# visinf/da-sac

Measured on AMD Instinct MI355X. Metric: train images/sec (769x769, 19-cls, RN101 DeepLabv2, K=3), higher is better.
Workload: dtype f32

## Files before the change

### da-sac_amd/csrc/conv_plan.hpp

```cpp
#pragma once
#include <cstddef>
#include <cstdint>

#include "chip.hpp"

#if defined(__HIPCC__)
#include <hip/hip_runtime.h>
#define DASAC_PLAN_HD __host__ __device__ __forceinline__
#else
#define DASAC_PLAN_HD inline
#endif

namespace dasac {

constexpr int kBK = 16;
constexpr int kSkWorkersPerCu = 3;
constexpr int kSkWorkers = kNumCu * kSkWorkersPerCu;
constexpr int kTileSlots = kNumCu * 4;
constexpr int kTailSlots = 2048;
constexpr int kTailMinSteps = 8;
constexpr double kTailPieceCost = 6.0;
constexpr int kTailMaxSplit = 8;
constexpr size_t kDepositBytes = (size_t)128 * 128 * sizeof(float);
constexpr size_t kPartialBytes = (size_t)(kTailSlots > kSkWorkers ? kTailSlots : kSkWorkers) * kDepositBytes;
constexpr size_t kGemmWorkspaceBytes = kPartialBytes + (size_t)(kTailSlots + 1) * sizeof(int);

constexpr int kWgPix = 32;
constexpr int kWgMinPix = 256;
constexpr int kWgSlots = kNumCu * 3;
constexpr int kWgMaxSplits = 64;
constexpr int kWgFewTiles = 12;
constexpr int kWgManyPix = 200000;
constexpr int64_t kMaxTensorBytes = (1ll << 32) - 4096;

inline int conv_mpad(int M) { return M > 64 ? (M + 127) / 128 * 128 : (M > 32 ? 64 : 32); }
inline int conv_kpad(int K) { return (K + 127) / 128 * 128; }
inline int pick_bm(int Mpad) { return Mpad % 128 == 0 ? 128 : (Mpad % 64 == 0 ? 64 : 32); }
DASAC_PLAN_HD int round_up_xcd(int n) { return (n + kNumXcd - 1) / kNumXcd * kNumXcd; }

inline int sk_workers(int reserved) { return (kNumCu - reserved) * kSkWorkersPerCu; }

inline bool want_streamk(int tiles, int k_steps, int reserved) {
  if ((long long)tiles * k_steps < sk_workers(reserved)) return false;
  const int resident = (kNumCu - reserved) * 3;
  const int rounds = (tiles + resident - 1) / resident;
  const double eff = (double)tiles / ((double)rounds * resident);
  return k_steps >= 64 ? eff < 0.93 : (k_steps >= 16 && eff < 0.6);
}

inline int tail_plan(int m_tiles, int n_tiles, int k_steps, int reserved, int& lead_n) {
  const int tiles = m_tiles * n_tiles;
  if (!want_streamk(tiles, k_steps, reserved)) return 0;
  lead_n = (tiles / kTileSlots) * kTileSlots / m_tiles;
// ... 95 lines not shown
  p.bm = pick_bm(p.Mpad);
  p.bnk = (M % 8 == 0 && p.bm != 32) ? wgrad_bn(Cx) : 128;
  p.m_tiles = p.Mpad / p.bm;
  p.k_tiles = p.Kpad / p.bnk;
  p.splits = wgrad_splits(p.Mpad, p.Kpad, Npix, p.bm, p.bnk);
  p.per = wgrad_per(Npix, p.splits);
  p.grid = round_up_xcd(p.m_tiles * p.k_tiles * p.splits);
  p.slab = (size_t)p.Mpad * p.Kpad;
  p.psum_offset = (size_t)p.splits * p.slab;
  const int s128 = wgrad_splits(p.Mpad, p.Kpad, Npix, p.bm, 128), s64 = wgrad_splits(p.Mpad, p.Kpad, Npix, p.bm, 64);
  p.workspace_bytes = (size_t)(s128 > s64 ? s128 : s64) * p.Mpad * (p.Kpad + 1) * sizeof(float);
  return p;
}

struct WgradBatchedPlan {
  int m_tiles, k_tiles, splits, per, grid;
  size_t psum_offset, workspace_bytes;
};
inline WgradBatchedPlan wgrad_batched_plan(int batch, int M, int C, int T) {
  WgradBatchedPlan p{};
  if (batch < 1 || batch > 65535 || M <= 0 || C <= 0 || T <= 0 || M % 128 || C % 128 || T % 4) return p;
  if ((int64_t)M * T * 4 >= (1ll << 31) || (int64_t)C * T * 4 >= (1ll << 31)) return p;
  if ((int64_t)batch * M * C * 4 > kMaxTensorBytes) return p;
  const int splits = wgrad_splits(batch * (M / 128) * (C / 128), T, kWgMaxSplits);
  if ((int64_t)splits * batch * M * C * 4 > kMaxTensorBytes) return p;
  p.m_tiles = M / 128;
  p.k_tiles = C / 128;
  p.splits = splits;
  p.per = wgrad_per(T, splits);
  p.grid = round_up_xcd(p.m_tiles * p.k_tiles * splits);
  p.psum_offset = (size_t)splits * batch * M * C;
  p.workspace_bytes = (size_t)splits * ((size_t)batch * M * C + M) * sizeof(float);
  return p;
}

struct GemmWork {
  bool has_work;
  int it, it_end;
};

DASAC_PLAN_HD GemmWork gemm_tile_work(int bid, int m_tiles, int n_tiles, int KT) {
  const int xcd = bid % kNumXcd, slot = bid / kNumXcd;
  const int per_xcd = (n_tiles + kNumXcd - 1) / kNumXcd;
  const int n_local = slot / m_tiles;
  const int n_tile = xcd * per_xcd + n_local;
  const int it = (n_tile * m_tiles + slot % m_tiles) * KT;
  return GemmWork{!(n_local >= per_xcd || n_tile >= n_tiles), it, it + KT};
// ... 25 lines not shown
```

### da-sac_amd/csrc/winograd.hip

```cpp
#include "conv_common.hpp"
#include "winograd_index.hpp"

namespace dasac {
namespace wino {

constexpr int kBlock = 256;

__device__ __forceinline__ float ld(__amdgpu_buffer_rsrc_t r, unsigned voff) {
  return __uint_as_float(__builtin_amdgcn_raw_buffer_load_b32(r, voff, 0, 0));
}
__device__ __forceinline__ void st(__amdgpu_buffer_rsrc_t r, unsigned voff, float v) {
  __builtin_amdgcn_raw_buffer_store_b32(__float_as_uint(v), r, voff, 0, 0);
}

struct F2 {
  static constexpr int TM = 2, N = TM + 2, P = kPoints<TM>;
  static constexpr bool kPaddedT = wino::kPaddedT<TM>;
  static __device__ __forceinline__ void bt(const float (&d)[4], float (&o)[4]) {
    o[0] = d[0] - d[2];
    o[1] = d[1] + d[2];
    o[2] = d[2] - d[1];
    o[3] = d[1] - d[3];
  }
  static __device__ __forceinline__ void a(const float (&y)[2], float (&o)[4]) {
// ... 33 lines not shown
    o[2] = (y[0] + y[2]) - (y[1] + y[3]);
    o[3] = (y[0] + 4.f * y[2]) + (2.f * y[1] + 8.f * y[3]);
    o[4] = (y[0] + 0.25f * y[2]) - (0.5f * y[1] + 0.125f * y[3]);
    o[5] = y[3];
  }
  static __device__ __forceinline__ void g(const float (&w)[3], float (&o)[6]) {
    o[0] = 0.5f * w[0];
    o[1] = k6 * ((w[0] + w[2]) + w[1]);
    o[2] = k6 * ((w[0] + w[2]) - w[1]);
    o[3] = (k30 * w[0] + k15 * w[1]) + (2.f * k15) * w[2];
    o[4] = ((16.f * k15) * w[0] - (8.f * k15) * w[1]) + (4.f * k15) * w[2];
    o[5] = 0.5f * w[2];
  }
  static __device__ __forceinline__ void gt(const float (&p)[6], float (&o)[3]) {
    o[0] = (0.5f * p[0] + k6 * (p[1] + p[2])) + (k30 * p[3] + (16.f * k15) * p[4]);
    o[1] = k6 * (p[1] - p[2]) + (k15 * p[3] - (8.f * k15) * p[4]);
    o[2] = (k6 * (p[1] + p[2]) + 0.5f * p[5]) + ((2.f * k15) * p[3] + (4.f * k15) * p[4]);
  }
  static __device__ __forceinline__ void at(const float (&y)[6], float (&o)[4]) {
    o[0] = (y[0] + (y[1] + y[2])) + (y[3] + y[4]);
    o[1] = (y[1] - y[2]) + (2.f * y[3] - 0.5f * y[4]);
    o[2] = (y[1] + y[2]) + (4.f * y[3] + 0.25f * y[4]);
    o[3] = ((y[1] - y[2]) + y[5]) + (8.f * y[3] - 0.125f * y[4]);
  }
};


template <class F>
__global__ __launch_bounds__(kBlock) void filter_transform(const float* __restrict__ Wt, const float* __restrict__ scale,
                                                            float* __restrict__ U, int Cout, int Cin, int Mpad, int Kpad, int mode,
                                                            unsigned w_bytes, unsigned u_bytes) {
  const int idx = blockIdx.x * kBlock + threadIdx.x;
  const int per_point = Kpad * Mpad;
  if (idx >= per_point) return;
  const __amdgpu_buffer_rsrc_t rw = make_rsrc(Wt, w_bytes), ru = make_rsrc(U, u_bytes);
  const int row4 = Mpad * 4;
  const int kq = idx / row4, rem = idx - kq * row4;
  const int m = rem >> 2, k = kq * 4 + (rem & 3);
  const int M = mode == 0 ? Cout : Cin, K = mode == 0 ? Cin : Cout;
  const bool real = m < M && k < K;
  const int co = mode == 0 ? m : k, ci = mode == 0 ? k : m;
  const float s = (real && scale) ? ld(make_rsrc(scale, (unsigned)Cout * 4u), (unsigned)co * 4u) : 1.f;
  float w[3][3];
#pragma unroll
  for (int a = 0; a < 3; ++a)
#pragma unroll
// ... 143 lines not shown
      float o[3];
      F::gt(r[a], o);
#pragma unroll
      for (int b = 0; b < 3; ++b) grad[c * 9 + a * 3 + b] = o[b];
    }
  }
  __syncthreads();
  const float sc = scale ? ld(make_rsrc(scale, (unsigned)M * 4u), (unsigned)co * 4u) : 1.f;
  float part = 0.f;
  for (int e = tx; e < 64 * 9; e += kBlock) {
    const unsigned off = ((unsigned)(co * C + ci0) * 9u + (unsigned)e) * 4u;
    if (dot) part += grad[e] * ld(rw, off);
    st(rd, off, grad[e] * sc);
  }
  if (dot) {
    __shared__ float redd[4];
    part = wave_sum(part);
    if (c == 0) redd[q] = part;
    __syncthreads();
    if (tx == 0) st(make_rsrc(dot, (unsigned)((C / 64) * M) * 4u), (unsigned)(blockIdx.x * M + co) * 4u, (redd[0] + redd[1]) + (redd[2] + redd[3]));
  }
}


__device__ __forceinline__ void record_bits(unsigned* obits, unsigned bits_bytes, int m, int w32, int pix, bool positive) {
  const unsigned long long ballot = __builtin_amdgcn_ballot_w64(positive);
  const int lane = threadIdx.x & 63, wcol = pix >> 5;
  if ((lane & 31) == 0 && wcol < w32)
    __builtin_amdgcn_raw_buffer_store_b32((unsigned)(lane ? ballot >> 32 : ballot), make_rsrc(obits, bits_bytes), out_bits_offset(m, w32, pix), 0, 0);
}

template <int BITS>
__global__ __launch_bounds__(kBlock) void output_transform(const float* __restrict__ Y, float* __restrict__ Out, Geom g, int M,
                                                            const float* __restrict__ shift, int relu,
                                                            const unsigned* __restrict__ mbits, unsigned* __restrict__ obits,
                                                            int w32, unsigned y_bytes, unsigned out_bytes, unsigned bits_bytes) {
  const int pix = blockIdx.x * kBlock + threadIdx.x;
  const int m = blockIdx.y;
  const bool live = pix < g.N * g.HW;
  const __amdgpu_buffer_rsrc_t ry = make_rsrc(Y, y_bytes), ro = make_rsrc(Out, out_bytes);
  int n = 0, rem = 0, tile = 0, ey = 0, ex = 0;
  if (live) pixel_tile(g, pix, n, rem, tile, ey, ex);
  float v[3][3];
#pragma unroll
  for (int j = 0; j < 3; ++j)
#pragma unroll
// ... 56 lines not shown
        v = (word >> (pix & 31)) & 1u ? v : 0.f;
      }
      st(ro, in ? out_offset(g, M, n, m, rem) : kOutside, v);
    }
  }
}

__global__ __launch_bounds__(kBlock) void relu_bits_pack(const float* __restrict__ Out, unsigned* __restrict__ obits, Geom g, int M,
                                                          int w32, unsigned out_bytes, unsigned bits_bytes) {
  const int pix = blockIdx.x * kBlock + threadIdx.x;
  const int m = blockIdx.y;
  const bool live = pix < g.N * g.HW;
  const int n = live ? div(pix, g.by_hw) : 0;
  const float v = ld(make_rsrc(Out, out_bytes), live ? out_offset(g, M, n, m, pix - n * g.HW) : kOutside);
  record_bits(obits, bits_bytes, m, w32, pix, live && v > 0.f);
}

}
}

using namespace dasac;
using dasac::wino::F2;
using dasac::wino::F4;
using dasac::wino::Geom;

template <class F>
static int wino_geom(Geom& g, const char* who, int Nb, int C, int H, int W, int dilation) {
  DASAC_REQUIRE(Nb > 0 && C > 0 && H > 0 && W > 0 && dilation > 0, "%s: bad geometry", who);
  DASAC_REQUIRE((int64_t)Nb * H * W < (1ll << 30), "%s: more than 2^30 pixels", who);
  g = wino::make_geom<F::TM>(Nb, H, W, dilation);
  DASAC_REQUIRE(F::P * (int64_t)C * g.T * 4 <= wino::kMaxBytes && (int64_t)C * Nb * H * W * 4 <= wino::kMaxBytes,
                "%s: a tensor exceeds the 4 GiB buffer-descriptor window", who);
  DASAC_REQUIRE(C <= 65535, "%s: more than 65535 channels", who);
  return DASAC_OK;
}

template <class F>
static int tiles_impl(int Nb, int H, int W, int dilation) {
  if (Nb <= 0 || H <= 0 || W <= 0 || dilation <= 0) return 0;
  const int64_t t = (int64_t)Nb * wino::make_axis<F::TM>(H, dilation).tiles * wino::make_axis<F::TM>(W, dilation).tiles;
  return t < (1ll << 30) ? (int)wino::padded_tiles<F::TM>(t) : 0;
}

template <class F>
static int filter_impl(const char* who, const float* w, const float* scale, int Cout, int Cin, int transposed, float* u,
                       dasac_stream_t stream) {
// ... 61 lines not shown
                         out_bytes, bits_bytes);
    if (relu_bits_out) {
      DASAC_CHECK_LAUNCH(who);
      hipLaunchKernelGGL(wino::relu_bits_pack, per_pixel, block, 0, s, out, relu_bits_out, g, M, w32, out_bytes, bits_bytes);
    }
  }
  DASAC_CHECK_LAUNCH(who);
  return DASAC_OK;
}

template <class F>
static int wgrad_finish_impl(const char* who, const void* workspace, size_t ws_bytes, int M, int C, int T, const float* w,
                             const float* scale, float* dw, float* dot, float* sum_dz, dasac_stream_t stream) {
  DASAC_REQUIRE(workspace && w && dw, "%s: null pointer", who);
  DASAC_REQUIRE(M > 0 && M <= 65535 && C > 0 && C % 64 == 0, "%s: needs 1..65535 output channels and a multiple of 64 input channels", who);
  const int splits = dasac_conv_wgrad_batched_splits(F::P, M, C, T);
  DASAC_REQUIRE(splits > 0, "%s: the batched weight-gradient launch does not take this shape", who);
  const size_t need = dasac_conv_wgrad_batched_workspace(F::P, M, C, T);
  if (ws_bytes < need) return fail(DASAC_EWORKSPACE, "%s: workspace too small (%zu < %zu)", who, ws_bytes, need);
  const int64_t s_elems = (int64_t)splits * F::P * M * C;
  DASAC_REQUIRE(s_elems * 4 <= wino::kMaxBytes && (int64_t)M * C * 9 * 4 <= wino::kMaxBytes,
                "%s: a tensor exceeds the 4 GiB buffer-descriptor window", who);
  const float* S = reinterpret_cast<const float*>(workspace);
  hipLaunchKernelGGL(wino::wgrad_finish<F>, dim3(C / 64, M), dim3(wino::kBlock), 0, as_stream(stream), S, S + s_elems, splits, M, C, w, scale,
                     dw, dot, sum_dz, (unsigned)(s_elems * 4), (unsigned)((int64_t)M * C * 9 * 4));
  DASAC_CHECK_LAUNCH(who);
  return DASAC_OK;
}

extern "C" int dasac_winograd_tiles(int Nb, int H, int W, int dilation) { return tiles_impl<F2>(Nb, H, W, dilation); }
extern "C" int dasac_winograd4_tiles(int Nb, int H, int W, int dilation) { return tiles_impl<F4>(Nb, H, W, dilation); }

extern "C" int dasac_winograd_filter(const float* w, const float* scale, int Cout, int Cin, int transposed, float* u,
                                     dasac_stream_t stream) {
  return filter_impl<F2>("winograd_filter", w, scale, Cout, Cin, transposed, u, stream);
}
extern "C" int dasac_winograd4_filter(const float* w, const float* scale, int Cout, int Cin, int transposed, float* u,
                                      dasac_stream_t stream) {
  return filter_impl<F4>("winograd4_filter", w, scale, Cout, Cin, transposed, u, stream);
}

extern "C" int dasac_winograd_input(const float* x, int Nb, int C, int H, int W, int dilation, float* v, size_t v_bytes,
                                    dasac_stream_t stream) {
  return transform_impl<F2>("winograd_input", wino::input_transform<F2>, x, Nb, C, H, W, dilation, v, v_bytes, stream);
}
extern "C" int dasac_winograd4_input(const float* x, int Nb, int C, int H, int W, int dilation, float* v, size_t v_bytes,
                                     dasac_stream_t stream) {
  return transform_impl<F4>("winograd4_input", wino::input_transform<F4>, x, Nb, C, H, W, dilation, v, v_bytes, stream);
}

extern "C" int dasac_winograd_grad_input(const float* dz, int Nb, int M, int H, int W, int dilation, float* dm, size_t dm_bytes,
                                         dasac_stream_t stream) {
  return transform_impl<F2>("winograd_grad_input", wino::grad_transform<F2>, dz, Nb, M, H, W, dilation, dm, dm_bytes, stream);
}
extern "C" int dasac_winograd4_grad_input(const float* dz, int Nb, int M, int H, int W, int dilation, float* dm, size_t dm_bytes,
                                          dasac_stream_t stream) {
  return transform_impl<F4>("winograd4_grad_input", wino::grad_transform<F4>, dz, Nb, M, H, W, dilation, dm, dm_bytes, stream);
}

extern "C" int dasac_winograd_output(const float* y, size_t y_bytes, int Nb, int M, int H, int W, int dilation, const float* shift,
                                     int relu, const uint32_t* mask_bits, uint32_t* relu_bits_out, float* out,
                                     dasac_stream_t stream) {
  return output_impl<F2>("winograd_output", y, y_bytes, Nb, M, H, W, dilation, shift, relu, mask_bits, relu_bits_out, out, stream);
}
extern "C" int dasac_winograd4_output(const float* y, size_t y_bytes, int Nb, int M, int H, int W, int dilation, const float* shift,
                                      int relu, const uint32_t* mask_bits, uint32_t* relu_bits_out, float* out,
                                      dasac_stream_t stream) {
  return output_impl<F4>("winograd4_output", y, y_bytes, Nb, M, H, W, dilation, shift, relu, mask_bits, relu_bits_out, out, stream);
}

extern "C" int dasac_winograd_wgrad_finish(const void* workspace, size_t ws_bytes, int M, int C, int T, const float* w,
                                           const float* scale, float* dw, float* dot, float* sum_dz, dasac_stream_t stream) {
  return wgrad_finish_impl<F2>("winograd_wgrad_finish", workspace, ws_bytes, M, C, T, w, scale, dw, dot, sum_dz, stream);
}
extern "C" int dasac_winograd4_wgrad_finish(const void* workspace, size_t ws_bytes, int M, int C, int T, const float* w,
                                            const float* scale, float* dw, float* dot, float* sum_dz, dasac_stream_t stream) {
  return wgrad_finish_impl<F4>("winograd4_wgrad_finish", workspace, ws_bytes, M, C, T, w, scale, dw, dot, sum_dz, stream);
}
```

### da-sac_amd/csrc/winograd_index.hpp

```cpp
#pragma once
#include <stdint.h>

#if defined(__HIPCC__)
#define DASAC_HD __host__ __device__ __forceinline__
#else
#define DASAC_HD inline
#endif

namespace dasac {
namespace wino {

struct Div {
  unsigned mul, shift;
  int d;
};
DASAC_HD Div make_div(int d) {
  Div f{0u, 0u, d < 1 ? 1 : d};
  if (d <= 1) return f;
  int l = 1;
  while ((1ll << l) < d) ++l;
  const unsigned long long p = 1ull << (31 + l);
  f.mul = (unsigned)((p + (unsigned)d - 1) / (unsigned)d);
  f.shift = (unsigned)(l - 1);
  return f;
}
DASAC_HD int div(int n, Div f) {
  return f.mul ? (int)((unsigned)(((unsigned long long)(unsigned)n * f.mul) >> 32) >> f.shift) : n;
}

template <int TM>
constexpr int kPoints = (TM + 2) * (TM + 2);
template <int TM>
constexpr bool kPaddedT = TM == 4;
template <int TM>
DASAC_HD int64_t padded_tiles(int64_t tiles) { return kPaddedT<TM> ? (tiles + 3) / 4 * 4 : tiles; }

struct Axis {
  int n, d;
  int q, r;
  int b;
  int full;
  int tiles;
  Div by_d;
};
template <int TM = 2>
DASAC_HD Axis make_axis(int n, int d) {
  static_assert(TM == 2 || TM == 4, "outputs per tile and axis: 2 or 4 (coord_to_tile shifts by log2)");
  Axis a;
  a.n = n;
  a.d = d;
  a.q = n / d;
  a.r = n - a.q * d;
  a.b = (a.q + TM - 1) / TM;
  a.full = a.b * d;
  a.tiles = a.full + ((a.q & (TM - 1)) == 0 ? a.r : 0);
  a.by_d = make_div(d);
  return a;
}
DASAC_HD int phase_samples(const Axis& a, int p) { return a.q + (p < a.r ? 1 : 0); }
DASAC_HD void tile_decode(const Axis& a, int g, int& p, int& t) {
  if (g < a.full) {
    t = div(g, a.by_d);
    p = g - t * a.d;
  } else {
    t = a.b;
    p = g - a.full;
  }
}
DASAC_HD int tile_encode(const Axis& a, int p, int t) { return t < a.b ? t * a.d + p : a.full + p; }
template <int TM = 2>
DASAC_HD int first_out(const Axis& a, int p, int t) { return p + TM * a.d * t; }
template <int TM = 2>
DASAC_HD void coord_to_tile(const Axis& a, int o, int& g, int& e) {
  const int i = div(o, a.by_d), p = o - i * a.d;
  e = i & (TM - 1);
  g = tile_encode(a, p, i >> (TM == 4 ? 2 : 1));
}

struct Geom {
  Axis ay, ax;
  int N, H, W, HW;
  int tiles_img;
  int T;
  Div by_tiles_img, by_tx, by_hw, by_w;
};
template <int TM = 2>
DASAC_HD Geom make_geom(int N, int H, int W, int d) {
  Geom g;
  g.ay = make_axis<TM>(H, d);
  g.ax = make_axis<TM>(W, d);
  g.N = N;
  g.H = H;
  g.W = W;
  g.HW = H * W;
  g.tiles_img = g.ay.tiles * g.ax.tiles;
  g.T = (int)padded_tiles<TM>(N * g.tiles_img);
  g.by_tiles_img = make_div(g.tiles_img);
  g.by_tx = make_div(g.ax.tiles);
  g.by_hw = make_div(g.HW);
// ... 41 lines not shown
```

### da-sac_amd/dasac_hip/lib.py

```python
import ctypes as C
import os

import torch

LIB_PATH = os.environ.get("DASAC_LIB") or os.path.join(os.path.dirname(os.path.abspath(__file__)), "libdasac_hip.so")

_p, _i, _l, _f, _sz = C.c_void_p, C.c_int, C.c_int64, C.c_float, C.c_size_t

PROTOTYPES = {
    "dasac_version": (_i, []),
    "dasac_last_error": (C.c_char_p, []),
    "dasac_device_info": (_i, [C.POINTER(_i), C.POINTER(_i), C.c_char_p, _sz]),
    "dasac_reserved_cus": (_i, []),
    "dasac_set_reserved_cus": (_i, [_i]),
    "dasac_pseudo_labels_workspace": (_sz, [_i, _i, _l]),
    "dasac_pseudo_labels": (_i, [_p, _p, _p, _f, _f, _i, _i, _l, _p, _p, _p, _p, _sz, _p]),
    "dasac_conv_mpad": (_i, [_i]),
    "dasac_conv_kpad": (_i, [_i]),
    "dasac_conv_table": (_i, [_p, _p, _p, _p, _i, _i, _i, _i, _i, _i, _p, _p]),
    "dasac_conv_pack": (_i, [_p, _p, _i, _i, _i, _i, _i, _i, _i, _p, _p]),
    "dasac_relu_bits_words": (_sz, [_i, _l]),
    "dasac_conv_gemm_bits_ok": (_i, [_i, _i]),
    "dasac_conv_gemm": (_i, [_p, _p, _p, _p] + [_i] * 12 + [_p, _p, _p, _p, _p, _i, _i, _i, _i, _p, _sz, _p]),
    "dasac_conv_gemm_batched": (_i, [_p, _p, _p, _p] + [_i] * 12 + [_i, _l, _l, _l, _p]),
# ... 50 lines not shown
    "dasac_bn_apply": (_i, [_p, _p, _p, _p, _i, _i, _i, _l, _p, _p]),
    "dasac_bn_bwd_reduce": (_i, [_p, _p, _p, _p, _i, _i, _l, _p, _p, _p, _p, _sz, _p]),
    "dasac_bn_train_finalize_tiles": (_i, [_p, _i, _i, C.c_double, _p, _p, _p, _p, _p, _f, _f, _i, _p, _p, _p, _p, _p]),
    "dasac_bn_tile_stats_reduce": (_i, [_p, _i, _i, _i, _p, _p]),
    "dasac_bn_train_apply_tiles": (_i, [_p, _p, _i, _i, C.c_double, _p, _p, _p, _p, _p, _f, _f, _p, _i, _i, _i, _l, _p, _p, _p, _p]),
    "dasac_bn_bwd_fused": (_i, [_p, _p, _p, _p, _p, C.c_double, _i, _i, _l, _p, _p, _p, _p, _sz, _p]),
    "dasac_conv_gemm_stats_ok": (_i, [_i, _i]),
    "dasac_conv_gemm_stats_tiles": (_i, [_i, _i, _i]),
    "dasac_conv_gemm_stats": (_i, [_p, _p, _p, _p] + [_i] * 12 + [_p, _p, _i, _i, _i, _i, _p, _sz, _p, _p]),
    "dasac_bn_bwd_apply": (_i, [_p, _p, _p, _p, _p, _p, C.c_double, _p, _i, _i, _l, _p, _p, _p, _p]),
    "dasac_winograd_tiles": (_i, [_i, _i, _i, _i]),
    "dasac_winograd_filter": (_i, [_p, _p, _i, _i, _i, _p, _p]),
    "dasac_winograd_input": (_i, [_p, _i, _i, _i, _i, _i, _p, _sz, _p]),
    "dasac_winograd_output": (_i, [_p, _sz, _i, _i, _i, _i, _i, _p, _i, _p, _p, _p, _p]),
    "dasac_winograd_grad_input": (_i, [_p, _i, _i, _i, _i, _i, _p, _sz, _p]),
    "dasac_conv_wgrad_batched_splits": (_i, [_i, _i, _i, _i]),
    "dasac_conv_wgrad_batched_workspace": (_sz, [_i, _i, _i, _i]),
    "dasac_conv_wgrad_batched": (_i, [_p, _p, _i, _i, _i, _i, _l, _l, _i, _p, _sz, _p]),
    "dasac_winograd_wgrad_finish": (_i, [_p, _sz, _i, _i, _i, _p, _p, _p, _p, _p, _p]),
    "dasac_winograd4_tiles": (_i, [_i, _i, _i, _i]),
    "dasac_winograd4_input": (_i, [_p, _i, _i, _i, _i, _i, _p, _sz, _p]),
    "dasac_winograd4_grad_input": (_i, [_p, _i, _i, _i, _i, _i, _p, _sz, _p]),
    "dasac_winograd4_wgrad_finish": (_i, [_p, _sz, _i, _i, _i, _p, _p, _p, _p, _p, _p]),
    "dasac_winograd4_filter": (_i, [_p, _p, _i, _i, _i, _p, _p]),
    "dasac_winograd4_output": (_i, [_p, _sz, _i, _i, _i, _i, _i, _p, _i, _p, _p, _p, _p]),
    "dasac_conv_pack_expanded":(_i, [_p, _i, _i, _i, _i, _i, _i, _i, _p, _p]),
    "dasac_tap_gather": (_i, [_p, _p, _p, _p, _p, _i, _i, _i, _p, _i, _i, _i, _p, _p]),
    "dasac_tap_scatter": (_i, [_p, _p, _p, _p, _p, _i, _i, _i, _i, _i, _i, _p, _p]),
    "dasac_conv_wgrad_finish_expanded": (_i, [_p, _i, _i, _i, _i, _i, _p, _i, _i, _i, _i, _p]),
    "dasac_pack_chunk_elems": (_i, []),
    "dasac_bn_fold_multi": (_i, [_p, _p, _i, _p]),
    "dasac_conv_pack_multi": (_i, [_p, _p, _i, _p]),
    "dasac_label_pad_mask": (_i, [_p, _p, _l, _i, _i, _p]),
    "dasac_dropout_planes": (_i, [C.c_uint64, C.c_uint64, _f, _l, _p, _p]),
    "dasac_iou_counts": (_i, [_p, _p, _i, _i, _l, _i, _p, _p]),
    "dasac_mask_counts": (_i, [_p, _p, _p, _p, _p, _p, _p, _i, _i, _l, _i, _p, _p]),
    "dasac_confusion_counts": (_i, [_p, _p, _p, _p, _p, _p, _i, _p, _i, _i, _l, _i, _p, _p, _i, _i, _p]),
    "dasac_view_consistency": (_i, [_p, _i, _i, _i, _l, _f, _p, _p, _p, _p]),
    "dasac_boundary_counts_workspace": (_sz, [_i, _i, _i, _i]),
    "dasac_boundary_counts": (_i, [_p, _p, _p, _p, _p, _p, _i, _p, _i, _i, _i, _i, _i, _i, _p, _p, _sz, _p]),
    "dasac_label_segments_workspace": (_sz, [_i, _i, _i]),
    "dasac_label_segments": (_i, [_p, _i, _i, _i, _i, _i, _i, _p, _p, _p, _sz, _p]),
    "dasac_segment_counts_workspace": (_sz, [_i, _i, _i, _i]),
    "dasac_segment_counts": (_i, [_p, _p, _p, _p, _p, _p, _i, _p, _i, _i, _i, _i, _i, _i, _p, _p, _sz, _p]),
    "dasac_segment_filter_workspace": (_sz, [_i, _i, _i]),
    "dasac_segment_filter": (_i, [_p, _i, _i, _i, _i, _i, _i, _i, _i, _p, _p, _sz, _p]),
    "dasac_crf_meanfield_workspace": (_sz, [_i, _i, _i, _i, _i]),
# ... 123 lines not shown
```

### da-sac_amd/dasac_hip/ops.py

```python
import os

import torch

from . import lib as L


def _c(t):
    return t if t.is_contiguous() else t.contiguous()


class _Profile:

    def __init__(self):
        self.on, self.records = False, []

    def start(self):
        self.on, self.records = True, []

    def stop(self, by_shape=False):
        self.on = False
        torch.cuda.synchronize()
        out = {}
        for name, flops, a, b, tag, nbytes in self.records:
            d = out.setdefault((name, tag) if by_shape else name, {"flops": 0.0, "bytes": 0.0, "seconds": 0.0, "launches": 0})
# ... 361 lines not shown
        v_elems, m_elems = P * C * T, P * M * T
        ws = L.workspace(4 * (v_elems + m_elems) + slab_bytes, x.device)
        v, dm, slabs = ws[:4 * v_elems], ws[4 * v_elems:4 * (v_elems + m_elems)], ws[4 * (v_elems + m_elems):]
        dz = _c(dz)
        with PROFILE.span(name + "_wgrad_input", 0.0, None, 4.0 * (x.numel() + v_elems)):
            L.check(self.entry("input")(x.data_ptr(), Nb, C, H, W, d, v.data_ptr(), v.numel(), L.stream_ptr()), "dasac_{}_input".format(name))
        with PROFILE.span(name + "_wgrad_grad", 0.0, None, 4.0 * (dz.numel() + m_elems)):
            L.check(self.entry("grad_input")(dz.data_ptr(), Nb, M, H, W, d, dm.data_ptr(), dm.numel(), L.stream_ptr()),
                    "dasac_{}_grad_input".format(name))
        with PROFILE.span(name + "_wgrad_gemm", 2.0 * P * M * C * T, (M, C, T, 1, 1, False, False), 4.0 * (v_elems + m_elems + P * M * C)):
            L.check(lib.dasac_conv_wgrad_batched(dm.data_ptr(), v.data_ptr(), P, M, C, T, M * T, C * T, self.sum_entry, slabs.data_ptr(),
                                                 slabs.numel(), L.stream_ptr()), "dasac_conv_wgrad_batched")
        dw = _dest(out, weight)
        with PROFILE.span(name + "_wgrad_finish", 0.0, None, float(slab_bytes) + 8.0 * weight.numel()):
            L.check(self.entry("wgrad_finish")(slabs.data_ptr(), slabs.numel(), M, C, T, _c(weight).data_ptr(), L.ptr(scale), dw.data_ptr(),
                                            L.ptr(dot), L.ptr(sum_dz), L.stream_ptr()), "dasac_{}_wgrad_finish".format(name))
        return dw


F2 = WinogradForm("winograd", 2, multi_launch=True)
F4 = WinogradForm("winograd4", 4, multi_launch=False)
winograd_filter, winograd_output, winograd_conv, winograd_wgrad = F2.filter, F2.output, F2.conv, F2.wgrad
winograd4_filter, winograd4_output, winograd4_conv, winograd4_wgrad = F4.filter, F4.output, F4.conv, F4.wgrad


def winograd_routed(spec, transposed, Nb, H, W):
    if ALGORITHM != "auto" or not winograd_ok(spec, transposed) or spec.cin * spec.cout < WINOGRAD_MIN_CHANNEL_PRODUCT:
        return False
    return F2.fits(spec.cin, spec.cout, F2.tiles(Nb, H, W, spec.branches[0][2]))


WINOGRAD4_ROUTES = {
    (512, 512, 4, True, True),
    (512, 512, 4, False, False),
    (256, 256, 2, False, False),
}
WINOGRAD4_MIN_SAMPLES = 8


def winograd4_routed(spec, transposed, Nb, H, W, grad):
    if ALGORITHM != "auto" or not winograd_ok(spec, transposed):
        return False
    d = spec.branches[0][2]
    if (spec.cin, spec.cout, d, bool(transposed), bool(grad)) not in WINOGRAD4_ROUTES:
        return False
    if L.load().dasac_conv_mpad(spec.cin if transposed else spec.cout) % 128:
# ... 12 lines not shown
WINOGRAD_WGRAD_MIN_CHANNEL_PRODUCT = 256 * 256
WINOGRAD4_WGRAD_LAYERS = {(256, 256), (512, 512)}


def winograd_wgrad_routed(spec, Nb, H, W):
    if ALGORITHM != "auto" or not winograd_ok(spec) or spec.cin * spec.cout < WINOGRAD_WGRAD_MIN_CHANNEL_PRODUCT:
        return False
    T = F2.tiles(Nb, H, W, spec.branches[0][2])
    return F2.fits(spec.cin, spec.cout, T) and L.load().dasac_conv_wgrad_batched_splits(F2.points, spec.cout, spec.cin, T) > 0


def winograd4_wgrad_routed(spec, Nb, H, W):
    if ALGORITHM != "auto" or not winograd_ok(spec) or spec.cin * spec.cout < WINOGRAD_WGRAD_MIN_CHANNEL_PRODUCT:
        return False
    if spec.cin % 128 or spec.cout % 128 or (spec.cin, spec.cout) not in WINOGRAD4_WGRAD_LAYERS:
        return False
    d = spec.branches[0][2]
    if H // d < WINOGRAD4_MIN_SAMPLES or W // d < WINOGRAD4_MIN_SAMPLES:
        return False
    T = F4.tiles(Nb, H, W, d)
    return F4.fits(spec.cin, spec.cout, T) and L.load().dasac_conv_wgrad_batched_splits(F4.points, spec.cout, spec.cin, T) > 0


def winograd_wgrad_form(spec, Nb, H, W):
    if winograd4_wgrad_routed(spec, Nb, H, W):
        return F4
    return F2 if winograd_wgrad_routed(spec, Nb, H, W) else None


def dot_rows(spec):
    return L.load().dasac_conv_wgrad_dot_rows(spec.cin, spec.taps)


def conv_wgrad(spec, dz, x, weights, scale=None, dot=None, table=None, sum_dz=None, outs=None):
    lib = L.load()
    L.require_gpu(dz, x, *weights)
    assert dot is None or (tuple(dot.shape) == (dot_rows(spec), spec.cout) and dot.is_contiguous())
    Nb, Cx, H, W = x.shape
    _, M, OH, OW = dz.shape
    table = conv_table(spec, H, W, False, x.device) if table is None else table
    nbytes = lib.dasac_conv_wgrad_workspace(Nb, OH, OW, M, spec.K)
    ws = L.workspace(nbytes, x.device)
    with PROFILE.span("conv_wgrad", 2.0 * Nb * OH * OW * M * spec.K, (M, spec.K, Nb * OH * OW, spec.stride, 1, False, False),
                      4.0 * (dz.numel() + x.numel() + M * spec.K)):
        fn = lib.dasac_conv_wgrad_x3 if PRECISION == "bf16x3" else lib.dasac_conv_wgrad
        L.check(fn(_c(dz).data_ptr(), x.data_ptr(), table.data_ptr(), Nb, Cx, H, W, OH, OW, spec.stride, M,
                   spec.K, ws.data_ptr(), ws.numel(), L.stream_ptr()), "dasac_conv_wgrad")
# ... 1128 lines not shown
```

### include/dasac_hip.h

```cpp
#ifndef DASAC_HIP_H
#define DASAC_HIP_H

#include <stddef.h>
#include <stdint.h>

#ifdef __cplusplus
extern "C" {
#endif

#define DASAC_OK 0
#define DASAC_EINVAL (-1)
#define DASAC_EWORKSPACE (-2)
#define DASAC_ELAUNCH (-3)

typedef void* dasac_stream_t;

int dasac_version(void);
const char* dasac_last_error(void);
int dasac_device_info(int* cu_count, int* wave_size, char* arch, size_t arch_len);
int dasac_reserved_cus(void);
int dasac_set_reserved_cus(int n);

size_t dasac_pseudo_labels_workspace(int B, int C, int64_t HW);
int dasac_pseudo_labels(const float* probs, const uint8_t* ignore, const float* disc,
// ... 58 lines not shown
int dasac_winograd_input(const float* x, int Nb, int C, int H, int W, int dilation, float* v, size_t v_bytes,
                         dasac_stream_t stream);
int dasac_winograd_output(const float* y, size_t y_bytes, int Nb, int M, int H, int W, int dilation, const float* shift,
                          int relu, const uint32_t* mask_bits, uint32_t* relu_bits_out, float* out, dasac_stream_t stream);
int dasac_winograd_grad_input(const float* dz, int Nb, int M, int H, int W, int dilation, float* dm, size_t dm_bytes,
                              dasac_stream_t stream);
int dasac_conv_wgrad_batched_splits(int batch, int M, int C, int T);
size_t dasac_conv_wgrad_batched_workspace(int batch, int M, int C, int T);
int dasac_conv_wgrad_batched(const float* a, const float* b, int batch, int M, int C, int T, int64_t a_stride, int64_t b_stride,
                             int sum_entry, void* workspace, size_t ws_bytes, dasac_stream_t stream);
int dasac_winograd_wgrad_finish(const void* workspace, size_t ws_bytes, int M, int C, int T, const float* w, const float* scale,
                                float* dw, float* dot, float* sum_dz, dasac_stream_t stream);
int dasac_winograd4_tiles(int Nb, int H, int W, int dilation);
int dasac_winograd4_input(const float* x, int Nb, int C, int H, int W, int dilation, float* v, size_t v_bytes,
                          dasac_stream_t stream);
int dasac_winograd4_grad_input(const float* dz, int Nb, int M, int H, int W, int dilation, float* dm, size_t dm_bytes,
                               dasac_stream_t stream);
int dasac_winograd4_wgrad_finish(const void* workspace, size_t ws_bytes, int M, int C, int T, const float* w, const float* scale,
                                 float* dw, float* dot, float* sum_dz, dasac_stream_t stream);
int dasac_winograd4_filter(const float* w, const float* scale, int Cout, int Cin, int transposed, float* u,
                           dasac_stream_t stream);
int dasac_winograd4_output(const float* y, size_t y_bytes, int Nb, int M, int H, int W, int dilation, const float* shift,
                           int relu, const uint32_t* mask_bits, uint32_t* relu_bits_out, float* out, dasac_stream_t stream);

int dasac_conv_pack_expanded(const float* w, int Cout, int Cin, int taps, int tap0, int total_taps,
                             int Cp, int transposed, float* packed, dasac_stream_t stream);
int dasac_tap_gather(const float* y, const int32_t* kh, const int32_t* kw, const int32_t* dil,
                     const int32_t* pad, int n_branches, int Cp, int Cout, const float* bias, int B,
                     int H, int W, float* out, dasac_stream_t stream);
int dasac_tap_scatter(const float* dout, const int32_t* kh, const int32_t* kw, const int32_t* dil,
                      const int32_t* pad, int n_branches, int Cp, int Cout, int B, int H, int W,
                      float* d, dasac_stream_t stream);
int dasac_conv_wgrad_finish_expanded(const void* workspace, int Nb, int OH, int OW, int E, int Cin,
                                     float* dw, int Cout, int taps, int tap0, int Cp,
                                     dasac_stream_t stream);

int dasac_upsample_softmax(const float* logits, int B, int C, int h, int w, int H, int W,
                           const uint8_t* ignore, float* up, float* probs, double* class_sums,
                           dasac_stream_t stream);
size_t dasac_upsample_bwd_workspace(int planes, int H, int w);
int dasac_upsample_bwd(const float* grad_up, int planes, int h, int w, int H, int W,
                       const float* gscale, float* grad_low, void* workspace, size_t ws_bytes,
                       dasac_stream_t stream);
size_t dasac_ce_loss_workspace(int B, int C, int64_t HW);
int dasac_ce_loss(const float* logits, const int64_t* labels, const float* class_weight,
                  const float* conf, int B, int C, int64_t HW, int mode, const float* gscale,
// ... 221 lines not shown
```

Measured before the change: 23.67.

## Add Winograd F(6x6,3x3) weight-gradient path for 256/512-channel 3x3 layers

Adds an F6 Winograd form with 8x8 tiles, covering the input, gradient and filter transforms and a multi-pass finish kernel that reduces the split partial sums. Weight gradients for 256x256 and 512x512 3x3 convolutions are routed through it ahead of F4, which cuts the number of transformed tiles and batched GEMM work. The batched wgrad planner also doubles the split count when the grid would fill only one round with short per-split work. The tradeoff is more transform arithmetic, 64 transform points instead of 36, and possibly worse fp32 numerical accuracy from the larger tile.

```diff
diff --git a/da-sac_amd/csrc/conv_plan.hpp b/da-sac_amd/csrc/conv_plan.hpp
--- a/da-sac_amd/csrc/conv_plan.hpp
+++ b/da-sac_amd/csrc/conv_plan.hpp
@@ -29,6 +29,7 @@
 constexpr int kWgMinPix = 256;
 constexpr int kWgSlots = kNumCu * 3;
 constexpr int kWgMaxSplits = 64;
+constexpr int kWgOneRoundSteps = 48;
 constexpr int kWgFewTiles = 12;
 constexpr int kWgManyPix = 200000;
 constexpr int64_t kMaxTensorBytes = (1ll << 32) - 4096;
@@ -170,7 +171,11 @@
   if (batch < 1 || batch > 65535 || M <= 0 || C <= 0 || T <= 0 || M % 128 || C % 128 || T % 4) return p;
   if ((int64_t)M * T * 4 >= (1ll << 31) || (int64_t)C * T * 4 >= (1ll << 31)) return p;
   if ((int64_t)batch * M * C * 4 > kMaxTensorBytes) return p;
-  const int splits = wgrad_splits(batch * (M / 128) * (C / 128), T, kWgMaxSplits);
+  const int tiles = batch * (M / 128) * (C / 128);
+  int splits = wgrad_splits(tiles, T, kWgMaxSplits);
+  if (tiles * splits <= kWgSlots && wgrad_per(T, splits) < kWgOneRoundSteps * kWgPix &&
+      2 * (int64_t)splits * kWgMinPix < (int64_t)T + kWgMinPix && 2 * splits <= kWgMaxSplits)
+    splits *= 2;
   if ((int64_t)splits * batch * M * C * 4 > kMaxTensorBytes) return p;
   p.m_tiles = M / 128;
   p.k_tiles = C / 128;
diff --git a/da-sac_amd/csrc/winograd.hip b/da-sac_amd/csrc/winograd.hip
--- a/da-sac_amd/csrc/winograd.hip
+++ b/da-sac_amd/csrc/winograd.hip
@@ -79,6 +79,55 @@
     o[1] = (y[1] - y[2]) + (2.f * y[3] - 0.5f * y[4]);
     o[2] = (y[1] + y[2]) + (4.f * y[3] + 0.25f * y[4]);
     o[3] = ((y[1] - y[2]) + y[5]) + (8.f * y[3] - 0.125f * y[4]);
+  }
+};
+
+struct F6 {
+  static constexpr int TM = 6, N = TM + 2, P = kPoints<TM>;
+  static constexpr bool kPaddedT = wino::kPaddedT<TM>;
+  static constexpr float k18 = 1.f / 18.f, k45 = 1.f / 45.f, k90 = 1.f / 90.f, k180 = 1.f / 180.f, k360 = 1.f / 360.f;
+  static __device__ __forceinline__ void bt(const float (&d)[8], float (&o)[8]) {
+    const float e1 = 17.f * d[4] - 4.f * (d[2] + d[6]), o1 = 17.f * d[3] - 4.f * (d[1] + d[5]);
+    const float e2 = (d[2] + 4.f * d[6]) - 5.f * d[4], o2 = (2.f * d[1] + 8.f * d[5]) - 10.f * d[3];
+    const float e3 = (8.f * d[2] + 2.f * d[6]) - 10.f * d[4], o3 = (4.f * d[1] + d[5]) - 5.f * d[3];
+    o[0] = 4.f * (d[0] - d[6]) + 21.f * (d[4] - d[2]);
+    o[1] = e1 + o1;
+    o[2] = e1 - o1;
+    o[3] = e2 + o2;
+    o[4] = e2 - o2;
+    o[5] = e3 + o3;
+    o[6] = e3 - o3;
+    o[7] = 4.f * (d[7] - d[1]) + 21.f * (d[3] - d[5]);
+  }
+  static __device__ __forceinline__ void a(const float (&y)[6], float (&o)[8]) {
+    const float e1 = (y[0] + y[2]) + y[4], o1 = (y[1] + y[3]) + y[5];
+    const float e2 = (y[0] + 4.f * y[2]) + 16.f * y[4], o2 = (2.f * y[1] + 8.f * y[3]) + 32.f * y[5];
+    const float e3 = (y[0] + 0.25f * y[2]) + 0.0625f * y[4], o3 = (0.5f * y[1] + 0.125f * y[3]) + 0.03125f * y[5];
+    o[0] = y[0];
+    o[1] = e1 + o1;
+    o[2] = e1 - o1;
+    o[3] = e2 + o2;
+    o[4] = e2 - o2;
+    o[5] = e3 + o3;
+    o[6] = e3 - o3;
+    o[7] = y[5];
+  }
+  static __device__ __forceinline__ void g(const float (&w)[3], float (&o)[8]) {
+    const float e1 = w[0] + w[2], e2 = k360 * w[0] + k90 * w[2], e3 = (16.f * k45) * w[0] + (4.f * k45) * w[2];
+    o[0] = 0.25f * w[0];
+    o[1] = k18 * (e1 + w[1]);
+    o[2] = k18 * (e1 - w[1]);
+    o[3] = e2 + k180 * w[1];
+    o[4] = e2 - k180 * w[1];
+    o[5] = e3 + (8.f * k45) * w[1];
+    o[6] = e3 - (8.f * k45) * w[1];
+    o[7] = 0.25f * w[2];
+  }
+  static __device__ __forceinline__ void gt(const float (&p)[8], float (&o)[3]) {
+    const float s1 = p[1] + p[2], t1 = p[1] - p[2], s2 = p[3] + p[4], t2 = p[3] - p[4], s3 = p[5] + p[6], t3 = p[5] - p[6];
+    o[0] = (0.25f * p[0] + k18 * s1) + (k360 * s2 + (16.f * k45) * s3);
+    o[1] = k18 * t1 + (k180 * t2 + (8.f * k45) * t3);
+    o[2] = (k18 * s1 + 0.25f * p[7]) + (k90 * s2 + (4.f * k45) * s3);
   }
 };
 
@@ -268,6 +317,80 @@
   }
 }
 
+template <class F, int NC>
+__global__ __launch_bounds__(kBlock) void wgrad_finish_passes(const float* __restrict__ S, const float* __restrict__ Ssum, int splits,
+                                                               int M, int C, const float* __restrict__ Wt,
+                                                               const float* __restrict__ scale, float* __restrict__ dW,
+                                                               float* __restrict__ dot, float* __restrict__ sum_dz, unsigned s_bytes,
+                                                               unsigned w_bytes) {
+  static_assert(F::N % NC == 0, "whole passes");
+  const int co = blockIdx.y, ci0 = blockIdx.x * 64;
+  const int tx = threadIdx.x, c = tx & 63, q = tx >> 6;
+  const __amdgpu_buffer_rsrc_t rp = make_rsrc(S, s_bytes), rw = make_rsrc(Wt, w_bytes), rd = make_rsrc(dW, w_bytes);
+  if (sum_dz && blockIdx.x == 0 && q == 0) {
+    const __amdgpu_buffer_rsrc_t rs = make_rsrc(Ssum, (unsigned)(splits * M) * 4u);
+    float sv = 0.f;
+    for (int s = c; s < splits; s += 64) sv += ld(rs, (unsigned)(s * M + co) * 4u);
+    sv = wave_sum(sv);
+    if (c == 0) st(make_rsrc(sum_dz, (unsigned)M * 4u), (unsigned)co * 4u, sv);
+  }
+  __shared__ float red[4][F::N * NC][64];
+  __shared__ float grad[64 * 9];
+  const unsigned point = (unsigned)(M * C), slab = (unsigned)F::P * point;
+  const unsigned e0 = (unsigned)(co * C + ci0 + c);
+  float r[3][F::N];
+#pragma unroll
+  for (int b0 = 0; b0 < F::N; b0 += NC) {
+    float acc[F::N * NC];
+#pragma unroll
+    for (int i = 0; i < F::N * NC; ++i) acc[i] = 0.f;
+    for (int s = q; s < splits; s += 4)
+#pragma unroll
+      for (int i = 0; i < F::N * NC; ++i)
+        acc[i] += ld(rp, ((unsigned)s * slab + (unsigned)((i / NC) * F::N + b0 + i % NC) * point + e0) * 4u);
+#pragma unroll
+    for (int i = 0; i < F::N * NC; ++i) red[q][i][c] = acc[i];
+    __syncthreads();
+    if (q == 0) {
+#pragma unroll
+      for (int j = 0; j < NC; ++j) {
+        float p[F::N], o[3];
+#pragma unroll
+        for (int a = 0; a < F::N; ++a)
+          p[a] = (red[0][a * NC + j][c] + red[1][a * NC + j][c]) + (red[2][a * NC + j][c] + red[3][a * NC + j][c]);
+        F::gt(p, o);
+#pragma unroll
+        for (int a = 0; a < 3; ++a) r[a][b0 + j] = o[a];
+      }
+    }
+    if (b0 + NC < F::N) __syncthreads();
+  }
+  if (q == 0) {
+#pragma unroll
+    for (int a = 0; a < 3; ++a) {
+      float o[3];
+      F::gt(r[a], o);
+#pragma unroll
+      for (int b = 0; b < 3; ++b) grad[c * 9 + a * 3 + b] = o[b];
+    }
+  }
+  __syncthreads();
+  const float sc = scale ? ld(make_rsrc(scale, (unsigned)M * 4u), (unsigned)co * 4u) : 1.f;
+  float part = 0.f;
+  for (int e = tx; e < 64 * 9; e += kBlock) {
+    const unsigned off = ((unsigned)(co * C + ci0) * 9u + (unsigned)e) * 4u;
+    if (dot) part += grad[e] * ld(rw, off);
+    st(rd, off, grad[e] * sc);
+  }
+  if (dot) {
+    __shared__ float redd[4];
+    part = wave_sum(part);
+    if (c == 0) redd[q] = part;
+    __syncthreads();
+    if (tx == 0) st(make_rsrc(dot, (unsigned)((C / 64) * M) * 4u), (unsigned)(blockIdx.x * M + co) * 4u, (redd[0] + redd[1]) + (redd[2] + redd[3]));
+  }
+}
+
 
 __device__ __forceinline__ void record_bits(unsigned* obits, unsigned bits_bytes, int m, int w32, int pix, bool positive) {
   const unsigned long long ballot = __builtin_amdgcn_ballot_w64(positive);
@@ -370,6 +493,7 @@
 using namespace dasac;
 using dasac::wino::F2;
 using dasac::wino::F4;
+using dasac::wino::F6;
 using dasac::wino::Geom;
 
 template <class F>
@@ -477,14 +601,21 @@
   DASAC_REQUIRE(s_elems * 4 <= wino::kMaxBytes && (int64_t)M * C * 9 * 4 <= wino::kMaxBytes,
                 "%s: a tensor exceeds the 4 GiB buffer-descriptor window", who);
   const float* S = reinterpret_cast<const float*>(workspace);
-  hipLaunchKernelGGL(wino::wgrad_finish<F>, dim3(C / 64, M), dim3(wino::kBlock), 0, as_stream(stream), S, S + s_elems, splits, M, C, w, scale,
-                     dw, dot, sum_dz, (unsigned)(s_elems * 4), (unsigned)((int64_t)M * C * 9 * 4));
+  const auto launch = [&](auto* kernel) {
+    hipLaunchKernelGGL(kernel, dim3(C / 64, M), dim3(wino::kBlock), 0, as_stream(stream), S, S + s_elems, splits, M, C, w, scale, dw, dot,
+                       sum_dz, (unsigned)(s_elems * 4), (unsigned)((int64_t)M * C * 9 * 4));
+  };
+  if constexpr (F::TM == 6)
+    launch(wino::wgrad_finish_passes<F, 4>);
+  else
+    launch(wino::wgrad_finish<F>);
   DASAC_CHECK_LAUNCH(who);
   return DASAC_OK;
 }
 
 extern "C" int dasac_winograd_tiles(int Nb, int H, int W, int dilation) { return tiles_impl<F2>(Nb, H, W, dilation); }
 extern "C" int dasac_winograd4_tiles(int Nb, int H, int W, int dilation) { return tiles_impl<F4>(Nb, H, W, dilation); }
+extern "C" int dasac_winograd6_tiles(int Nb, int H, int W, int dilation) { return tiles_impl<F6>(Nb, H, W, dilation); }
 
 extern "C" int dasac_winograd_filter(const float* w, const float* scale, int Cout, int Cin, int transposed, float* u,
                                      dasac_stream_t stream) {
@@ -503,6 +634,10 @@
                                      dasac_stream_t stream) {
   return transform_impl<F4>("winograd4_input", wino::input_transform<F4>, x, Nb, C, H, W, dilation, v, v_bytes, stream);
 }
+extern "C" int dasac_winograd6_input(const float* x, int Nb, int C, int H, int W, int dilation, float* v, size_t v_bytes,
+                                     dasac_stream_t stream) {
+  return transform_impl<F6>("winograd6_input", wino::input_transform<F6>, x, Nb, C, H, W, dilation, v, v_bytes, stream);
+}
 
 extern "C" int dasac_winograd_grad_input(const float* dz, int Nb, int M, int H, int W, int dilation, float* dm, size_t dm_bytes,
                                          dasac_stream_t stream) {
@@ -511,6 +646,10 @@
 extern "C" int dasac_winograd4_grad_input(const float* dz, int Nb, int M, int H, int W, int dilation, float* dm, size_t dm_bytes,
                                           dasac_stream_t stream) {
   return transform_impl<F4>("winograd4_grad_input", wino::grad_transform<F4>, dz, Nb, M, H, W, dilation, dm, dm_bytes, stream);
+}
+extern "C" int dasac_winograd6_grad_input(const float* dz, int Nb, int M, int H, int W, int dilation, float* dm, size_t dm_bytes,
+                                          dasac_stream_t stream) {
+  return transform_impl<F6>("winograd6_grad_input", wino::grad_transform<F6>, dz, Nb, M, H, W, dilation, dm, dm_bytes, stream);
 }
 
 extern "C" int dasac_winograd_output(const float* y, size_t y_bytes, int Nb, int M, int H, int W, int dilation, const float* shift,
@@ -532,3 +671,7 @@
                                             const float* scale, float* dw, float* dot, float* sum_dz, dasac_stream_t stream) {
   return wgrad_finish_impl<F4>("winograd4_wgrad_finish", workspace, ws_bytes, M, C, T, w, scale, dw, dot, sum_dz, stream);
 }
+extern "C" int dasac_winograd6_wgrad_finish(const void* workspace, size_t ws_bytes, int M, int C, int T, const float* w,
+                                            const float* scale, float* dw, float* dot, float* sum_dz, dasac_stream_t stream) {
+  return wgrad_finish_impl<F6>("winograd6_wgrad_finish", workspace, ws_bytes, M, C, T, w, scale, dw, dot, sum_dz, stream);
+}
diff --git a/da-sac_amd/csrc/winograd_index.hpp b/da-sac_amd/csrc/winograd_index.hpp
--- a/da-sac_amd/csrc/winograd_index.hpp
+++ b/da-sac_amd/csrc/winograd_index.hpp
@@ -31,7 +31,7 @@
 template <int TM>
 constexpr int kPoints = (TM + 2) * (TM + 2);
 template <int TM>
-constexpr bool kPaddedT = TM == 4;
+constexpr bool kPaddedT = TM != 2;
 template <int TM>
 DASAC_HD int64_t padded_tiles(int64_t tiles) { return kPaddedT<TM> ? (tiles + 3) / 4 * 4 : tiles; }
 
@@ -45,7 +45,7 @@
 };
 template <int TM = 2>
 DASAC_HD Axis make_axis(int n, int d) {
-  static_assert(TM == 2 || TM == 4, "outputs per tile and axis: 2 or 4 (coord_to_tile shifts by log2)");
+  static_assert(TM == 2 || TM == 4 || TM == 6, "outputs per tile and axis: 2, 4 or 6");
   Axis a;
   a.n = n;
   a.d = d;
@@ -53,7 +53,7 @@
   a.r = n - a.q * d;
   a.b = (a.q + TM - 1) / TM;
   a.full = a.b * d;
-  a.tiles = a.full + ((a.q & (TM - 1)) == 0 ? a.r : 0);
+  a.tiles = a.full + (a.q % TM == 0 ? a.r : 0);
   a.by_d = make_div(d);
   return a;
 }
@@ -73,8 +73,14 @@
 template <int TM = 2>
 DASAC_HD void coord_to_tile(const Axis& a, int o, int& g, int& e) {
   const int i = div(o, a.by_d), p = o - i * a.d;
-  e = i & (TM - 1);
-  g = tile_encode(a, p, i >> (TM == 4 ? 2 : 1));
+  if constexpr (TM == 6) {
+    const int t = i / 6;
+    e = i - 6 * t;
+    g = tile_encode(a, p, t);
+  } else {
+    e = i & (TM - 1);
+    g = tile_encode(a, p, i >> (TM == 4 ? 2 : 1));
+  }
 }
 
 struct Geom {
diff --git a/da-sac_amd/dasac_hip/lib.py b/da-sac_amd/dasac_hip/lib.py
--- a/da-sac_amd/dasac_hip/lib.py
+++ b/da-sac_amd/dasac_hip/lib.py
@@ -96,7 +96,11 @@
     "dasac_winograd4_input": (_i, [_p, _i, _i, _i, _i, _i, _p, _sz, _p]),
     "dasac_winograd4_grad_input": (_i, [_p, _i, _i, _i, _i, _i, _p, _sz, _p]),
     "dasac_winograd4_wgrad_finish": (_i, [_p, _sz, _i, _i, _i, _p, _p, _p, _p, _p, _p]),
-    "dasac_winograd4_filter": (_i, [_p, _p, _i, _i, _i, _p, _p]),
+    "dasac_winograd6_tiles": (_i, [_i, _i, _i, _i]),
+    "dasac_winograd6_input": (_i, [_p, _i, _i, _i, _i, _i, _p, _sz, _p]),
+    "dasac_winograd6_grad_input": (_i, [_p, _i, _i, _i, _i, _i, _p, _sz, _p]),
+    "dasac_winograd6_wgrad_finish": (_i, [_p, _sz, _i, _i, _i, _p, _p, _p, _p, _p, _p]),
+    "dasac_winograd4_filter":(_i, [_p, _p, _i, _i, _i, _p, _p]),
     "dasac_winograd4_output": (_i, [_p, _sz, _i, _i, _i, _i, _i, _p, _i, _p, _p, _p, _p]),
     "dasac_conv_pack_expanded":(_i, [_p, _i, _i, _i, _i, _i, _i, _i, _p, _p]),
     "dasac_tap_gather": (_i, [_p, _p, _p, _p, _p, _i, _i, _i, _p, _i, _i, _i, _p, _p]),
diff --git a/da-sac_amd/dasac_hip/ops.py b/da-sac_amd/dasac_hip/ops.py
--- a/da-sac_amd/dasac_hip/ops.py
+++ b/da-sac_amd/dasac_hip/ops.py
@@ -407,6 +407,8 @@
 F4 = WinogradForm("winograd4", 4, multi_launch=False)
 winograd_filter, winograd_output, winograd_conv, winograd_wgrad = F2.filter, F2.output, F2.conv, F2.wgrad
 winograd4_filter, winograd4_output, winograd4_conv, winograd4_wgrad = F4.filter, F4.output, F4.conv, F4.wgrad
+F6 = WinogradForm("winograd6", 6, multi_launch=False)
+winograd6_wgrad = F6.wgrad
 
 
 def winograd_routed(spec, transposed, Nb, H, W):
@@ -465,7 +467,25 @@
     return F4.fits(spec.cin, spec.cout, T) and L.load().dasac_conv_wgrad_batched_splits(F4.points, spec.cout, spec.cin, T) > 0
 
 
+WINOGRAD6_WGRAD_LAYERS = {(256, 256), (512, 512)}
+WINOGRAD6_MIN_SAMPLES = 12
+
+
+def winograd6_wgrad_routed(spec, Nb, H, W):
+    if ALGORITHM != "auto" or not winograd_ok(spec) or spec.cin * spec.cout < WINOGRAD_WGRAD_MIN_CHANNEL_PRODUCT:
+        return False
+    if spec.cin % 128 or spec.cout % 128 or (spec.cin, spec.cout) not in WINOGRAD6_WGRAD_LAYERS:
+        return False
+    d = spec.branches[0][2]
+    if H // d < WINOGRAD6_MIN_SAMPLES or W // d < WINOGRAD6_MIN_SAMPLES:
+        return False
+    T = F6.tiles(Nb, H, W, d)
+    return F6.fits(spec.cin, spec.cout, T) and L.load().dasac_conv_wgrad_batched_splits(F6.points, spec.cout, spec.cin, T) > 0
+
+
 def winograd_wgrad_form(spec, Nb, H, W):
+    if winograd6_wgrad_routed(spec, Nb, H, W):
+        return F6
     if winograd4_wgrad_routed(spec, Nb, H, W):
         return F4
     return F2 if winograd_wgrad_routed(spec, Nb, H, W) else None
diff --git a/include/dasac_hip.h b/include/dasac_hip.h
--- a/include/dasac_hip.h
+++ b/include/dasac_hip.h
@@ -104,6 +104,13 @@
                            dasac_stream_t stream);
 int dasac_winograd4_output(const float* y, size_t y_bytes, int Nb, int M, int H, int W, int dilation, const float* shift,
                            int relu, const uint32_t* mask_bits, uint32_t* relu_bits_out, float* out, dasac_stream_t stream);
+int dasac_winograd6_tiles(int Nb, int H, int W, int dilation);
+int dasac_winograd6_input(const float* x, int Nb, int C, int H, int W, int dilation, float* v, size_t v_bytes,
+                          dasac_stream_t stream);
+int dasac_winograd6_grad_input(const float* dz, int Nb, int M, int H, int W, int dilation, float* dm, size_t dm_bytes,
+                               dasac_stream_t stream);
+int dasac_winograd6_wgrad_finish(const void* workspace, size_t ws_bytes, int M, int C, int T, const float* w, const float* scale,
+                                 float* dw, float* dot, float* sum_dz, dasac_stream_t stream);
 
 int dasac_conv_pack_expanded(const float* w, int Cout, int Cin, int taps, int tap0, int total_taps,
                              int Cp, int transposed, float* packed, dasac_stream_t stream);
```

Result: no change. 23.86, median of 6 (+0.8%).
